# MasterXiong/Hyper-VLA

Hardware: AMD Instinct MI355X
Metric: actions_per_sec (higher is better)
Workload: dtype f16; 1 GPU; BASELINE configs[1]: hypernet weight-gen once (untimed) + full sample_actions step (u8 224x224 -> DINOv2-base E=768 in the loop -> generated vit_t 4L/64d policy -> [4,7] action chunk); 1 action = 1 sample-step; batch_per_gpu=256, global_batch=256, encoder=DINOv2-base (reference parity, E=768), parallelism=episode-dp1 (no collectives), policy_operands=split-bf16 (bf16x3), launch=eager (114 launches per step, counted by the library), streams=1, ensemble=not in the step

## Files before the change

hyper-vla_amd/csrc/api.hip:

```cpp
#include <hip/hip_runtime.h>

#include <cmath>
#include <cstdio>
#include <cstring>
#include <map>
#include <memory>
#include <mutex>
#include <string>
#include <vector>

#include "../../include/hvla.h"
#include "common.h"
#include "kernels.h"
#include "layout.h"
#include "pack.h"
#include "t5.h"
#include "train.h"

using namespace hvla;

namespace {

struct DevBuf {
  void* p = nullptr;
// ... 19 lines not shown
  DevBuf slot_count;
};

struct hvla_post {
  int B = 0, H = 0;
  DevBuf ring;
  DevBuf state;
};

struct hvla_ctx {
  hvla_config cfg{};
  Geom g{};
  int device = 0;
  std::string err;
  bool loaded = false;
  bool train_timer = false;
  PackedLayout lay;
  int Kp = 0;
  DevBuf hn_f32;
  CtxParams ctxp{};
  DevBuf wcat_hi, wcat_lo, bcat, perm;
  DevBuf enc16, encd16, encf32;
  EncWeights encw{};
  DevBuf ctx_hi, ctx_lo, ctx_f32, ws_x, ws_h, ws_qkv, ws_g, ws_corr, ws_abar, ws_lncnt, ws_lnpart, tokens, flags;
  uint32_t ln_spin = 800;
#ifdef HVLA_BENCH_HOOKS
  int enc_stop = 0;
#endif
  Profiler prof;
  float *amap_dino = nullptr, *amap_head = nullptr;
  hipStream_t side = nullptr;
  hipEvent_t ev_fork = nullptr, ev_join = nullptr;
  std::vector<hvla_weights*> arena_pool;
  std::mutex pool_mu;
  static constexpr size_t ARENA_POOL_MAX = 4;
  hipEvent_t ev_bucket[3] = {nullptr, nullptr, nullptr};
  bool bucket_recorded[3] = {false, false, false};
  ~hvla_ctx() {
    for (hvla_weights* w : arena_pool) delete w;
    for (hipEvent_t e : ev_bucket)
      if (e) (void)hipEventDestroy(e);
    if (ev_fork) (void)hipEventDestroy(ev_fork);
    if (ev_join) (void)hipEventDestroy(ev_join);
    if (side) (void)hipStreamDestroy(side);
  }
  int rs_H = 0, rs_W = 0, rs_row_span = 0, rs_col_span = 0;
  DevBuf rs_tab, rs_rows, rs_img, rs_pad;
  bool t5_loaded = false;
  T5Dims t5d{};
// ... 59 lines not shown
  ctx->Kp = 2 * ((g.patch * g.patch * 3 + 63) / 64 * 64);
  {
    std::vector<uint8_t> seen(ctx->lay.pl.G, 0);
    for (int32_t r : ctx->lay.perm)
      if (r >= 0) {
        if (r >= ctx->lay.pl.G || seen[r]) return HVLA_E_STATE;
        seen[r] = 1;
      }
    for (uint8_t s : seen)
      if (!s) return HVLA_E_STATE;
  }
  const size_t Bm = c->max_batch, S = g.S(), E = g.E, F = g.enc_mlp;
  size_t gbytes = Bm * S * F * 2;
  if (gbytes < Bm * P * ctx->Kp * 2) gbytes = Bm * P * ctx->Kp * 2;
  hipError_t e = hipSuccess;
  auto A = [&](DevBuf& b, size_t n) { if (e == hipSuccess) e = b.alloc(n); };
  A(ctx->ctx_hi, Bm * g.C * 2); A(ctx->ctx_lo, Bm * g.C * 2); A(ctx->ctx_f32, Bm * g.C * 4);
  A(ctx->ws_x, Bm * S * E * 4); A(ctx->ws_h, Bm * S * E * 2); A(ctx->ws_qkv, Bm * S * 3 * E * 2);
  A(ctx->ws_g, gbytes); A(ctx->tokens, Bm * P * E * 4); A(ctx->flags, 64 * sizeof(int));
  A(ctx->ws_corr, 2 * Bm * (F > 3 * E ? F : 3 * E) * 4);
  A(ctx->ws_abar, 2 * Bm * (F > E ? F : E) * 2);
  A(ctx->ws_lncnt, (Bm + 4) * 4 + 64);
  A(ctx->ws_lnpart, Bm * 4 * 256 * 16);
  if (e != hipSuccess) return HVLA_E_ARENA_FULL;
  if (hipMemset(ctx->ws_lncnt.p, 0, ctx->ws_lncnt.bytes) != hipSuccess) return HVLA_E_HIP;
  if (c->streams == 2) {
    if (hipStreamCreateWithFlags(&ctx->side, hipStreamNonBlocking) != hipSuccess ||
        hipEventCreateWithFlags(&ctx->ev_fork, hipEventDisableTiming) != hipSuccess ||
        hipEventCreateWithFlags(&ctx->ev_join, hipEventDisableTiming) != hipSuccess)
      return HVLA_E_HIP;
  } else if (c->streams != 0 && c->streams != 1) {
    return HVLA_E_SHAPE;
  }
  *out = ctx.release();
  return HVLA_OK;
}

void hvla_destroy(hvla_ctx* ctx) {
  if (!ctx) return;
  (void)hipSetDevice(ctx->device);
  if (ctx->train_timer) train_gemm_timer_release();
  delete ctx;
}

int64_t hvla_num_generated(const hvla_ctx* ctx) { return ctx ? ctx->lay.pl.G : 0; }

// ... 300 lines not shown
  if (context)
    HIPCHK(ctx, hipMemcpyAsync(context, w->ctx.p, (size_t)w->B * ctx->g.C * 4, hipMemcpyDeviceToDevice, st));
  return HVLA_OK;
}

static int check_step(hvla_ctx* ctx, int32_t B) {
  if (!ctx->loaded) FAIL(ctx, HVLA_E_STATE, "called before hvla_load_weights");
  if (B < 1 || B > ctx->cfg.max_batch) FAIL(ctx, HVLA_E_SHAPE, "batch %d outside [1, %d]", B, ctx->cfg.max_batch);
  return HVLA_OK;
}

static int encode_range(hvla_ctx* ctx, const uint8_t* images, float* out, int b0, int nb, bool keep_cls, hipStream_t st) {
  const Geom& g = ctx->g;
  const size_t S = g.S(), E = g.E, F = g.enc_mlp, rows = (size_t)b0 * S;
  const size_t gper = S * F > (size_t)g.P() * ctx->Kp ? S * F : (size_t)g.P() * ctx->Kp;
  EncWorkspace ws{ctx->ws_x.as<float>() + rows * E, static_cast<char*>(ctx->ws_h.p) + rows * E * 2,
                  static_cast<char*>(ctx->ws_qkv.p) + rows * 3 * E * 2, static_cast<char*>(ctx->ws_g.p) + (size_t)b0 * gper * 2,
                  ctx->ws_corr.as<float>() + (size_t)2 * b0 * (F > 3 * E ? F : 3 * E),
                  static_cast<char*>(ctx->ws_abar.p) + (size_t)2 * b0 * (F > E ? F : E) * 2};
  if (ctx->amap_dino) ws.amap = ctx->amap_dino + (size_t)b0 * g.enc_layers * g.enc_heads * g.P();
  ws.ln_cnt = ctx->ws_lncnt.as<uint32_t>() + (size_t)((b0 + 3) / 4 * 4);
  ws.ln_part = ctx->ws_lnpart.as<float>() + (size_t)b0 * 4 * 256 * 4;
  ws.ln_spin = ctx->ln_spin;
#ifdef HVLA_BENCH_HOOKS
  ws.stop_after = ctx->enc_stop;
#endif
  const size_t img = (size_t)g.image_size * g.image_size * 3, per = (keep_cls ? S : (size_t)g.P()) * E;
  HIPCHK(ctx, launch_encoder(g, ctx->cfg.enc_dtype, ctx->encw, ws, images + (size_t)b0 * img, out + (size_t)b0 * per, nb, st,
                             &ctx->prof, keep_cls));
  return HVLA_OK;
}

int hvla_encode(hvla_ctx* ctx, const uint8_t* images, float* tokens, int32_t B, void* stream) {
  if (!ctx) return HVLA_E_STATE;
  if (int r = check_step(ctx, B)) return r;
  if (!images || !tokens) FAIL(ctx, HVLA_E_SHAPE, "null pointer");
  HIPCHK(ctx, hipSetDevice(ctx->device));
  return encode_range(ctx, images, tokens, 0, B, false, reinterpret_cast<hipStream_t>(stream));
}

int hvla_encode_hidden(hvla_ctx* ctx, const uint8_t* images, float* hidden, int32_t B, void* stream) {
  if (!ctx) return HVLA_E_STATE;
  if (int r = check_step(ctx, B)) return r;
  if (!images || !hidden) FAIL(ctx, HVLA_E_SHAPE, "null pointer");
  HIPCHK(ctx, hipSetDevice(ctx->device));
  return encode_range(ctx, images, hidden, 0, B, true, reinterpret_cast<hipStream_t>(stream));
}

int hvla_encode_audit(hvla_ctx* ctx, const uint8_t* images, int32_t B, float* maxabs, int32_t* nonfinite, void* stream) {
  if (!ctx) return HVLA_E_STATE;
  if (int r = check_step(ctx, B)) return r;
  if (!images || !maxabs || !nonfinite) FAIL(ctx, HVLA_E_SHAPE, "null pointer");
  HIPCHK(ctx, hipSetDevice(ctx->device));
  hipStream_t st = reinterpret_cast<hipStream_t>(stream);
  uint32_t* slots = reinterpret_cast<uint32_t*>(ctx->flags.p);
  HIPCHK(ctx, hipMemsetAsync(slots, 0, 8 * sizeof(uint32_t), st));
  const Geom& g = ctx->g;
  const size_t F = g.enc_mlp, E = g.E;
  EncWorkspace ws{ctx->ws_x.as<float>(), ctx->ws_h.p, ctx->ws_qkv.p, ctx->ws_g.p, ctx->ws_corr.as<float>(), ctx->ws_abar.p};
  (void)F; (void)E;
  ws.ln_cnt = ctx->ws_lncnt.as<uint32_t>(); ws.ln_part = ctx->ws_lnpart.as<float>(); ws.ln_spin = ctx->ln_spin;
  HIPCHK(ctx, launch_encoder(g, ctx->cfg.enc_dtype, ctx->encw, ws, images, ctx->tokens.as<float>(), B, st, nullptr, false, slots));
  uint32_t h[8];
  HIPCHK(ctx, hipMemcpyAsync(h, slots, sizeof h, hipMemcpyDeviceToHost, st));
  HIPCHK(ctx, hipStreamSynchronize(st));
  for (int i = 0; i < 4; ++i) {
    memcpy(&maxabs[i], &h[2 * i], 4);
    nonfinite[i] = (int32_t)h[2 * i + 1];
  }
  return HVLA_OK;
}

static int policy_range(hvla_ctx* ctx, const hvla_weights* w, const float* tokens, float* actions, float* logits, int b0,
                        int nb, hipStream_t st, const int32_t* slots = nullptr) {
  const Geom& g = ctx->g;
  const PolicyLayout& pl = ctx->lay.pl;
  const size_t wb = slots ? 0 : (size_t)b0;
  PolicyParams p{pl, w->wh.as<__bf16>() + wb * pl.Gm, w->wl.as<__bf16>() + wb * pl.Gm,
                 w->vf.as<float>() + wb * pl.Gv, tokens + (size_t)b0 * g.P() * g.E,
                 actions + (size_t)b0 * g.horizon * g.action_dim, logits ? logits + (size_t)b0 * g.horizon : nullptr,
                 nb, g.E, g.P(), g.L, g.M, g.horizon, g.action_dim, g.tanh_scale, g.max_action};
  const LangLayout& ll = ctx->lay.ll;
  const int lang_T = ll.on ? g.T : 0;
  if (ctx->amap_head) p.amap = ctx->amap_head + (size_t)b0 * g.L * g.H * (g.P() + lang_T);
// ... 541 lines not shown
  HIPCHK(ctx, hipMemset(st.p, 0, (size_t)n * 8));
  PolicyParams p{pl, w->wh.as<__bf16>(), w->wl.as<__bf16>(), w->vf.as<float>(), tokens, actions, logits,
                 B, g.E, g.P(), g.L, g.M, g.horizon, g.action_dim, g.tanh_scale, g.max_action};
  p.stamps = st.as<unsigned long long>();
  for (int i = 0; i < 3; ++i) HIPCHK(ctx, launch_policy(p, nullptr));
  HIPCHK(ctx, hipDeviceSynchronize());
  HIPCHK(ctx, hipMemcpy(out, st.p, (size_t)n * 8, hipMemcpyDeviceToHost));
  return HVLA_OK;
}

int hvla_debug_train_gemm_exact(int on) {
  set_train_gemm_exact(on != 0);
  return HVLA_OK;
}
int hvla_debug_ctx_stamps(unsigned long long* out) { return debug_ctx_stamps(out) == hipSuccess ? HVLA_OK : HVLA_E_HIP; }
int hvla_debug_workspace(hvla_ctx* ctx, int which, void** ptr, size_t* bytes) {
  if (!ctx || !ptr || !bytes) return HVLA_E_STATE;
  DevBuf* b[8] = {&ctx->ws_x, &ctx->ws_h, &ctx->ws_qkv, &ctx->ws_g, &ctx->ws_corr, &ctx->ws_abar, &ctx->ws_lncnt, &ctx->ws_lnpart};
  if (which < 0 || which > 7) return HVLA_E_SHAPE;
  *ptr = b[which]->p;
  *bytes = b[which]->bytes;
  return HVLA_OK;
}
int hvla_debug_lnx_stats(hvla_ctx* ctx, unsigned long long* out, int reset) {
  if (!ctx) return HVLA_E_STATE;
  HIPCHK(ctx, hipSetDevice(ctx->device));
  HIPCHK(ctx, debug_lnx_stats(out, reset));
  return HVLA_OK;
}
int hvla_debug_encode_stop(hvla_ctx* ctx, int32_t n) {
  if (!ctx || n < 0) return HVLA_E_STATE;
  ctx->enc_stop = n;
  return HVLA_OK;
}
int hvla_debug_lnx_spin(hvla_ctx* ctx, uint32_t ticks) {
  if (!ctx) return HVLA_E_STATE;
  ctx->ln_spin = ticks;
  return HVLA_OK;
}
#endif

int64_t hvla_launches(hvla_ctx* ctx) {
  if (!ctx) return 0;
  const int64_t n = (int64_t)ctx->prof.nlaunch;
  ctx->prof.nlaunch = 0;
  return n;
// ... 29 lines not shown
```

hyper-vla_amd/csrc/encoder.hip:

```cpp
#include <cstring>
#include <type_traits>

#include "common.h"
#include "kernels.h"
#include "plan.h"

namespace hvla {

template <typename Op>
__global__ void im2col_kernel(const uint8_t* __restrict__ img, typename Op::elem* __restrict__ out, int B,
                              int image, int patch, int grid, int Kp, float* __restrict__ x, const float* __restrict__ pos, int S, int E) {
  for (size_t i = (size_t)blockIdx.x * blockDim.x + threadIdx.x; i < (size_t)B * E; i += (size_t)gridDim.x * blockDim.x)
    x[(i / E) * S * E + (i % E)] = pos[i % E];
  const int Kp1 = Kp / 2, chunks = Kp1 / 8;
  const size_t total = (size_t)B * grid * grid * chunks;
  const int kreal = patch * patch * 3;
  for (size_t i = (size_t)blockIdx.x * blockDim.x + threadIdx.x; i < total; i += (size_t)gridDim.x * blockDim.x) {
    const int ch = (int)(i % chunks);
    const size_t m = i / chunks;
    const int px = (int)(m % grid), py = (int)((m / grid) % grid);
    const size_t b = m / ((size_t)grid * grid);
    typename Op::x8 v;
    const int rowb = 3 * patch;
    const int k0 = ch * 8;
// ... 1856 lines not shown
    }
    o[((size_t)b * S + (S - 1)) * E + head * 64 + lane] = (T)last;
    if (omean) {
      const int NH = NW / 2;
      float t0 = 0.f, t1 = last;
      if (NW == 8) {
        float c[8];
#pragma unroll
        for (int w = 0; w < 8; ++w) c[w] = csum[w * 64 + lane];
#pragma unroll
        for (int w = 0; w < 4; ++w) t0 += c[w], t1 += c[4 + w];
      } else {
        for (int w = 0; w < NH; ++w) t0 += csum[w * 64 + lane];
        for (int w = NH; w < NW; ++w) t1 += csum[w * 64 + lane];
      }
      if (NH == 0) t0 = t1;
      omean[((size_t)b * 2 + 0) * E + head * 64 + lane] = (T)(t0 / (float)(NH ? NH * 32 : S));
      omean[((size_t)b * 2 + 1) * E + head * 64 + lane] = (T)(t1 / (float)(NH ? S - NH * 32 : S));
    }
  }
  HVLA_ASTAMP();
}

template <typename T>
__global__ __launch_bounds__(256) void colmean_kernel(const T* __restrict__ a, T* __restrict__ abar, int S, int P, int K) {
  typedef T T8 __attribute__((ext_vector_type(8)));
  __shared__ float part[8][256];
  const int b = blockIdx.y, chain = threadIdx.x >> 5, l32 = threadIdx.x & 31;
  const int wm = chain >> 2, pq = chain & 3;
  const int n0 = blockIdx.x * 256 + l32 * 8;
  const int half = P / 2, nq = half / 4;
  T8 p;
#pragma unroll
  for (int i = 0; i < 8; ++i) p[i] = (T)0.f;
  if (n0 < K) {
    const T* base = a + ((size_t)b * S + 1 + wm * half) * K + n0;
    for (int q = pq; q < nq; q += 16) {
      T8 v[4][4];
#pragma unroll
      for (int u = 0; u < 4; ++u)
        if (q + 4 * u < nq) {
#pragma unroll
          for (int r = 0; r < 4; ++r) v[u][r] = *reinterpret_cast<const T8*>(base + (size_t)(4 * (q + 4 * u) + r) * K);
        }
#pragma unroll
      for (int u = 0; u < 4; ++u)
// ... 49 lines not shown

#define HVLA_LAUNCH(...) do { ++pf.nlaunch; hipLaunchKernelGGL(__VA_ARGS__); } while (0)
template <typename Op>
static hipError_t run_encoder(const Geom& g, const EncWeights& w, const EncWorkspace& ws, const uint8_t* images,
                              float* tokens, int B, hipStream_t st, Profiler* prof, bool keep_cls, uint32_t* audit) {
  Profiler none;
  Profiler& pf = prof ? *prof : none;
  using T = typename Op::elem;
  constexpr int opi = std::is_same<Op, OpBF16>::value ? 1 : 0;
  const int P = g.P(), S = g.S(), E = g.E, F = g.enc_mlp, H = g.enc_heads;
  const int Kp = 2 * ((g.patch * g.patch * 3 + 63) / 64 * 64);
  const int M = B * S;
  if ((size_t)M * (size_t)(F > 3 * E ? F : 3 * E) >= (1ull << 32)) return hipErrorInvalidValue;
  const size_t gsm = (size_t)2 * (GBM + GBN) * GLD * sizeof(T);
  int dev = 0;
  hipError_t e = hipGetDevice(&dev);
  if (e != hipSuccess) return e;
  if (dev < 0 || dev >= 64) return hipErrorInvalidDevice;
  DeviceInfo& di = g_dev[dev];
  if (!di.attr[opi]) {
#define SETA(K) \
  if ((e = hipFuncSetAttribute(reinterpret_cast<const void*>(K), hipFuncAttributeMaxDynamicSharedMemorySize, 160 * 1024)) != hipSuccess) return e;
    SETA((gemm_kernel<Op, EPI_PATCH>)) SETA((gemm_kernel<Op, EPI_QKV>)) SETA((gemm_kernel<Op, EPI_GELU>))
    SETA((gemm_kernel<Op, EPI_RES>)) SETA((attention_kernel<Op, false>)) SETA((attention_kernel<Op, true>)) SETA((attention_kernel<Op, false, 8>))
    SETA((gemm256p_kernel<Op, EPI_PATCH, false>)) SETA((gemm256p_kernel<Op, EPI_QKV, false>))
    SETA((gemm256p_kernel<Op, EPI_GELU, false>)) SETA((gemm256p_kernel<Op, EPI_RES, false>))
    SETA((gemm256p_kernel<Op, EPI_PATCH, true>)) SETA((gemm256p_kernel<Op, EPI_QKV, true>))
    SETA((gemm256p_kernel<Op, EPI_GELU, true>)) SETA((gemm256p_kernel<Op, EPI_RES, true>))
    SETA((gemm256p_kernel<Op, EPI_PATCH, false, true>)) SETA((gemm256p_kernel<Op, EPI_RES, false, true>))
    SETA((gemm256p_kernel<Op, EPI_PATCH, true, true>)) SETA((gemm256p_kernel<Op, EPI_RES, true, true>))
    SETA((gemm256p_kernel<Op, EPI_RES, false, true, true>)) SETA((gemm256p_kernel<Op, EPI_RES, true, true, true>))
    SETA((gemm64_kernel<Op, EPI_PATCH>)) SETA((gemm64_kernel<Op, EPI_QKV>)) SETA((gemm64_kernel<Op, EPI_GELU>))
    SETA((gemm64_kernel<Op, EPI_RES>)) SETA((gemm64_kernel<Op, EPI_CORR>))
    SETA((gemm64_kernel<Op, EPI_QKV, 4>)) SETA((gemm64_kernel<Op, EPI_GELU, 4>)) SETA((gemm64_kernel<Op, EPI_RES, 4>))
    SETA((gemm64c_kernel<Op, EPI_QKV>)) SETA((gemm64c_kernel<Op, EPI_GELU>)) SETA((gemm64c_kernel<Op, EPI_RES>)) SETA((gemm64c32_kernel<Op>))
    SETA((gemm64c_kernel<Op, EPI_QKV, true>)) SETA((gemm64c_kernel<Op, EPI_GELU, true>)) SETA((layernorm_group_kernel<Op>))
    SETA((gemm256p_kernel<Op, EPI_QKV, false, false, true>)) SETA((gemm256p_kernel<Op, EPI_GELU, false, false, true>))
    SETA((gemm256p_kernel<Op, EPI_QKV, true, false, true>)) SETA((gemm256p_kernel<Op, EPI_GELU, true, false, true>))
    SETA((gemm256p_kernel<Op, EPI_RES, false, false, true>)) SETA((gemm256p_kernel<Op, EPI_RES, true, false, true>))
#undef SETA
    di.attr[opi] = true;
  }
  if (!di.ncu && (hipDeviceGetAttribute(&di.ncu, hipDeviceAttributeMultiprocessorCount, dev) != hipSuccess || di.ncu <= 0)) di.ncu = 256;
  const int ncu = di.ncu;
  constexpr int G64_MAXM = 2047;
  constexpr int CAT_COMP = 8;
  const bool comp = w.layer[0].dqkv != nullptr && ws.corr && ws.abar;
// ... 125 lines not shown
    float* partial = comp && room ? reinterpret_cast<float*>(scratch) : nullptr;
    HVLA_LAUNCH((layernorm_group_kernel<Op>), dim3(LNG, B), dim3(LNW * 64), (size_t)(P / 8) * E * sizeof(float), st, ws.x,
                       reinterpret_cast<T*>(ws.h), sc, bi, partial, S, P, E);
    if (!partial) return;
    if (small_fused(Nnext, E) && gemm64c_fold_lds(E) <= 160 * 1024 && ((M + SBM - 1) / SBM) * (Nnext / SBN) <= ncu) {
      ln_partial = partial;
      return;
    }
    HVLA_LAUNCH((layernorm_mean_kernel<Op>), dim3(2 * B), dim3(256), 0, st, partial, reinterpret_cast<T*>(ws.abar), P, E);
  };
  auto colmean_of = [&](const void* act, int K) {
    if (!comp) return;
    HVLA_LAUNCH((colmean_kernel<T>), dim3((K + 255) / 256, B), dim3(256), 0, st, reinterpret_cast<const T*>(act),
                       reinterpret_cast<T*>(ws.abar), S, P, K);
  };
  auto audit_of = [&](const void* buf, size_t n, int site) {
    if (!audit) return;
    HVLA_LAUNCH((absmax_kernel<T>), dim3(1024), dim3(256), 0, st, reinterpret_cast<const T*>(buf), n / 8, audit + 2 * site);
  };
  if (can_fuse_ln && P == HBM_ && M > G64_MAXM) {
    if ((e = hipMemsetAsync(ws.ln_cnt, 0, (size_t)((B * 4 + 15) / 16 * 16), st)) != hipSuccess) return e;
    if ((e = hipMemsetAsync(ws.ln_part, 0, (size_t)B * ((E + HBN_ - 1) / HBN_) * 256 * 16, st)) != hipSuccess) return e;
    pf.nlaunch += 2;
  }
  using EQ = std::integral_constant<int, EPI_QKV>;
  using EG = std::integral_constant<int, EPI_GELU>;
  using ER = std::integral_constant<int, EPI_RES>;
  pf.begin(0, st);
  {
    const size_t total = (size_t)B * P * (Kp / 16);
    int blocks = (int)((total + 255) / 256);
    if (blocks > 8192) blocks = 8192;
    HVLA_LAUNCH(im2col_kernel<Op>, dim3(blocks), dim3(256), 0, st, images, reinterpret_cast<T*>(ws.g), B,
                       g.image_size, g.patch, g.grid(), Kp, ws.x, w.pos, S, E);
    const int Mp = B * P;
    GemmArgs a{ws.g, w.w_patch, Mp, E, Kp, w.b_patch, w.pos, ws.x, P, S, 0, 1.f / 256.f};
    const bool fits32 = (size_t)Mp * Kp < (1ull << 31);
    if (Mp % HBM_ == 0 && E % SBN == 0 && E >= HBN_ && Mp > G64_MAXM && fits32) {
      a.nbm = Mp / HBM_; a.tile_row0 = 0; a.tile_stride = HBM_;
      const int nbn = (E + HBN_ - 1) / HBN_;
      if (P == HBM_ && can_fuse_ln && g.enc_layers > 0) {
        a.hsplit = hsplit;
        lnx_args(a, w.layer[0].ln1_s, w.layer[0].ln1_b, nbn);
        if (lnx_persistent(a.nbm, nbn)) HVLA_LAUNCH((gemm256p_kernel<Op, EPI_PATCH, true, true>), dim3(ncu), dim3(512), 131072, st, a);
        else HVLA_LAUNCH((gemm256p_kernel<Op, EPI_PATCH, false, true>), dim3(a.nbm * nbn), dim3(512), 131072, st, a);
        ln_fused = true;
// ... 19 lines not shown
    const EncLayerW& L = w.layer[l];
    if (!ln_fused) {
      pf.begin(1, st);
      layernorm(L.ln1_s, L.ln1_b, 3 * E, ws.g, F);
      pf.end(1, st);
    }
    audit_of(ws.h, (size_t)M * E, 0);
    gemm(EQ{}, ws.h, L.wqkv, L.dqkv, 3 * E, E, L.bqkv, nullptr, ws.qkv, E, 2);
    audit_of(ws.qkv, (size_t)M * 3 * E, 1);
    HVLA_STOP_HERE();
    pf.begin(3, st);
    const bool att_unrolled = KT == 9;
    auto attn = [&](auto kern, size_t lds) {
      HVLA_LAUNCH(kern, dim3(B * H), dim3((KT - 1) * 64), lds, st, reinterpret_cast<const T*>(ws.qkv), reinterpret_cast<T*>(ws.h), S, E, H,
                  comp ? reinterpret_cast<T*>(ws.abar) : nullptr, ws.amap ? ws.amap + (size_t)l * H * (S - 1) : nullptr, g.enc_layers * H * (S - 1)
#ifdef HVLA_BENCH_HOOKS
                  , (unsigned long long*)nullptr, 0
#endif
                  );
    };
    if (ws.amap) {
      attn(attention_kernel<Op, true>, asm_bytes + (size_t)(KT * 32 + 32) * sizeof(float));
    } else {
      if (att_unrolled) attn(attention_kernel<Op, false, 8>, asm_bytes);
      else attn(attention_kernel<Op, false>, asm_bytes);
    }
    pf.end(3, st);
    audit_of(ws.h, (size_t)M * E, 2);
    gemm(ER{}, ws.h, L.wo, L.dwo, E, E, L.bo, L.ls1, ws.x, 0, 4, nullptr, L.ln2_s, L.ln2_b);
    if (!ln_fused) {
      pf.begin(1, st);
      layernorm(L.ln2_s, L.ln2_b, F, ws.qkv, 3 * E);
      pf.end(1, st);
    }
    HVLA_STOP_HERE();
    audit_of(ws.h, (size_t)M * E, 0);
    const bool summed = gemm(EG{}, ws.h, L.w1, L.dw1, F, E, L.b1, nullptr, ws.g, 0, 5, comp ? ws.abar : nullptr);
    audit_of(ws.g, (size_t)M * F, 3);
    if (!summed) colmean_of(ws.g, F);
    HVLA_STOP_HERE();
    if (l + 1 < g.enc_layers) gemm(ER{}, ws.g, L.w2, L.dw2, E, F, L.b2, L.ls2, ws.x, 0, 6, nullptr, w.layer[l + 1].ln1_s, w.layer[l + 1].ln1_b);
    else gemm(ER{}, ws.g, L.w2, L.dw2, E, F, L.b2, L.ls2, ws.x, 0, 6);
    HVLA_STOP_HERE();
  }
#undef HVLA_STOP_HERE
  pf.begin(1, st);
  if (keep_cls)
// ... 41 lines not shown
    else if (variant == 2) hipLaunchKernelGGL((gemm256p_kernel<Op, EPI, false>), dim3(nt), dim3(512), 131072, st, a);
    else hipLaunchKernelGGL((gemm256p_kernel<Op, EPI, true>), dim3(nt < ncu ? nt : ncu), dim3(512), 131072, st, a);
  };
  auto launch = [&]() {
    if (epi == EPI_QKV) launch_e(std::integral_constant<int, EPI_QKV>{});
    else if (epi == EPI_GELU) launch_e(std::integral_constant<int, EPI_GELU>{});
    else launch_e(std::integral_constant<int, EPI_RES>{});
  };
  hipEvent_t e0, e1;
  (void)hipEventCreate(&e0);
  (void)hipEventCreate(&e1);
  launch();
  (void)hipEventRecord(e0, st);
  for (int i = 0; i < iters; ++i) launch();
  (void)hipEventRecord(e1, st);
  (void)hipEventSynchronize(e1);
  (void)hipEventElapsedTime(ms, e0, e1);
  *ms /= iters;
  (void)hipEventDestroy(e0);
  (void)hipEventDestroy(e1);
  return hipGetLastError();
}
hipError_t debug_attention_stamps(const void* qkv, void* o, void* omean, int B, int S, int E, int H, int wg, unsigned long long* stamps,
                                  hipStream_t st) {
  using Op = OpF16;
  using T = Op::elem;
  const int KT = (S + 31) / 32;
  const size_t asm_bytes = (size_t)KT * 32 * 2 * AVLD * sizeof(T) + (size_t)KT * APS * sizeof(float) + 64 * sizeof(T) +
                           (size_t)(KT - 1) * 64 * sizeof(float);
  auto go = [&](auto kern) {
    (void)hipFuncSetAttribute(reinterpret_cast<const void*>(kern), hipFuncAttributeMaxDynamicSharedMemorySize, 160 * 1024);
    hipLaunchKernelGGL(kern, dim3(B * H), dim3((KT - 1) * 64), asm_bytes, st, reinterpret_cast<const T*>(qkv),
                       reinterpret_cast<T*>(o), S, E, H, reinterpret_cast<T*>(omean), (float*)nullptr, 0, stamps, wg);
  };
  if (KT == 9) go(attention_kernel<Op, false, 8>);
  else go(attention_kernel<Op, false>);
  return hipGetLastError();
}
#endif

hipError_t launch_encoder(const Geom& g, int dtype, const EncWeights& w, const EncWorkspace& ws,
                          const uint8_t* images, float* tokens, int B, hipStream_t st, Profiler* prof, bool keep_cls,
                          uint32_t* audit) {
  if (dtype == 1) return run_encoder<OpBF16>(g, w, ws, images, tokens, B, st, prof, keep_cls, audit);
  return run_encoder<OpF16>(g, w, ws, images, tokens, B, st, prof, keep_cls, audit);
}

}
```

hyper-vla_amd/csrc/kernels.h:

```cpp
#pragma once
#include <hip/hip_runtime.h>
#include <stdint.h>

#include <vector>

#include "../../include/hvla.h"
#include "layout.h"

namespace hvla {

struct CtxLayer {
  const float *ln0_s, *ln0_b, *wq, *bq, *wk, *bk, *wv, *bv, *wo, *bo, *ln1_s, *ln1_b, *w1, *b1, *w2, *b2;
};
constexpr int CTX_MAX_LAYERS = 8;
struct CtxParams {
  int T, C, F, heads, layers, lang_dim, E, scale_context;
  int big_elems;
  const float* tok;
  const int64_t* attn_mask;
  const float* cls;
  const float *w_tok, *b_tok, *w_img, *b_img, *pos_tok, *pos_img, *pos_layer, *norm_s, *norm_b;
  CtxLayer layer[CTX_MAX_LAYERS];
  float* ctx;
  __bf16 *ctx_hi, *ctx_lo;
// ... 19 lines not shown
  const void *wqkv, *wo, *w1, *w2;
  const void *dqkv, *dwo, *dw1, *dw2;
  const float *bqkv, *bo, *b1, *b2;
  const float *ln1_s, *ln1_b, *ln2_s, *ln2_b, *ls1, *ls2;
};
constexpr int ENC_MAX_LAYERS = 24;
struct EncWeights {
  const void* w_patch;
  const float* b_patch;
  const float* pos;
  const float *lnf_s, *lnf_b;
  EncLayerW layer[ENC_MAX_LAYERS];
};
struct EncWorkspace {
  float* x;
  void* h;
  void* qkv;
  void* g;
  float* corr;
  void* abar;
  float* amap = nullptr;
  uint32_t* ln_cnt = nullptr;
  float* ln_part = nullptr;
  uint32_t ln_spin = 800;
#ifdef HVLA_BENCH_HOOKS
  int stop_after = 0;
#endif
};
struct Profiler {
  int mode = 0;
  uint32_t select = 1u << 5;
  std::vector<hipEvent_t> start, stop;
  std::vector<int> cat;
  size_t used = 0;
  uint64_t nlaunch = 0;
  bool want(int c) const { return c >= 0 && (mode == 2 || (mode == 1 && ((select >> c) & 1u))); }
  void begin(int c, hipStream_t st) {
    if (!want(c)) return;
    if (used == start.size()) {
      hipEvent_t a, b;
      if (hipEventCreate(&a) != hipSuccess || hipEventCreate(&b) != hipSuccess) return;
      start.push_back(a), stop.push_back(b), cat.push_back(c);
    }
    cat[used] = c;
    (void)hipEventRecord(start[used], st);
  }
  void end(int c, hipStream_t st) {
    if (!want(c) || used >= start.size()) return;
    (void)hipEventRecord(stop[used], st);
    ++used;
  }
};
hipError_t launch_encoder(const Geom& g, int dtype, const EncWeights& w, const EncWorkspace& ws,
                          const uint8_t* images, float* tokens, int B, hipStream_t st, Profiler* prof,
                          bool keep_cls = false,
                          uint32_t* audit = nullptr);

#ifdef HVLA_BENCH_HOOKS
hipError_t debug_gemm(const void* A, const void* W, const float* bias, const float* aux, void* out, int M, int N,
                      int K, int epi, int variant, int iters, float* ms, hipStream_t st);
hipError_t debug_lnx_stats(unsigned long long* out, int reset);
hipError_t debug_ctx_stamps(unsigned long long* out);
hipError_t debug_attention_stamps(const void* qkv, void* o, void* omean, int B, int S, int E, int H, int wg, unsigned long long* stamps,
                                  hipStream_t st);
#endif

void build_resize_spans(int in_size, int out_size, std::vector<int>& start, std::vector<int>& count, std::vector<float>& w,
                        int& maxspan);
hipError_t launch_resize(const uint8_t* src, uint8_t* dst, float* tmp_rows, float* tmp_img, const int* row_start,
                         const int* row_count, const float* row_w, int row_span, const int* col_start, const int* col_count,
                         const float* col_w, int col_span, int B, int H, int W, int S, int crop, hipStream_t st,
                         float* padded = nullptr, int src_h = 0, int src_w = 0);

struct PolicyParams {
  PolicyLayout pl;
  const __bf16 *wh, *wl;
  const float* vf;
  const float* tokens;
  float* actions;
  float* logits;
  int B, E, P, L, M, horizon, action_dim;
  float tanh_scale, max_action;
  float* amap = nullptr;
#ifdef HVLA_BENCH_HOOKS
  unsigned long long* stamps = nullptr;
#endif
};
// ... 44 lines not shown
```

Before: 18670 actions/s.

## Add persistent work-queue attention kernel overlapping next item's K/V loads

Adds a persistent DINOv2 attention kernel that launches at most two workgroups per CU. Each workgroup pulls (batch, head) items from an atomic ticket queue and prefetches the next item's Q/K/V into LDS while it computes the current one. The kernel is used by default when S==257, there is no attention-map capture, and B*H exceeds the slot count. The goal is to remove per-workgroup launch and tail overhead and hide global load latency. In exchange it adds one memset launch per encode, hand-tuned vmcnt waits and inline asm that are fragile, and an always-present queue buffer.

```diff
diff --git a/hyper-vla_amd/csrc/api.hip b/hyper-vla_amd/csrc/api.hip
--- a/hyper-vla_amd/csrc/api.hip
+++ b/hyper-vla_amd/csrc/api.hip
@@ -65,9 +65,10 @@
   DevBuf wcat_hi, wcat_lo, bcat, perm;
   DevBuf enc16, encd16, encf32;
   EncWeights encw{};
-  DevBuf ctx_hi, ctx_lo, ctx_f32, ws_x, ws_h, ws_qkv, ws_g, ws_corr, ws_abar, ws_lncnt, ws_lnpart, tokens, flags;
+  DevBuf ctx_hi, ctx_lo, ctx_f32, ws_x, ws_h, ws_qkv, ws_g, ws_corr, ws_abar, ws_lncnt, ws_lnpart, ws_attq, tokens, flags;
   uint32_t ln_spin = 800;
 #ifdef HVLA_BENCH_HOOKS
+  int att_form = 0;
   int enc_stop = 0;
 #endif
   Profiler prof;
@@ -173,6 +174,7 @@
   A(ctx->ws_abar, 2 * Bm * (F > E ? F : E) * 2);
   A(ctx->ws_lncnt, (Bm + 4) * 4 + 64);
   A(ctx->ws_lnpart, Bm * 4 * 256 * 16);
+  A(ctx->ws_attq, 2 * ENC_MAX_LAYERS * sizeof(uint32_t));
   if (e != hipSuccess) return HVLA_E_ARENA_FULL;
   if (hipMemset(ctx->ws_lncnt.p, 0, ctx->ws_lncnt.bytes) != hipSuccess) return HVLA_E_HIP;
   if (c->streams == 2) {
@@ -519,8 +521,10 @@
   ws.ln_cnt = ctx->ws_lncnt.as<uint32_t>() + (size_t)((b0 + 3) / 4 * 4);
   ws.ln_part = ctx->ws_lnpart.as<float>() + (size_t)b0 * 4 * 256 * 4;
   ws.ln_spin = ctx->ln_spin;
+  ws.att_queue = ctx->ws_attq.as<uint32_t>() + (b0 ? ENC_MAX_LAYERS : 0);
 #ifdef HVLA_BENCH_HOOKS
   ws.stop_after = ctx->enc_stop;
+  ws.att_form = ctx->att_form;
 #endif
   const size_t img = (size_t)g.image_size * g.image_size * 3, per = (keep_cls ? S : (size_t)g.P()) * E;
   HIPCHK(ctx, launch_encoder(g, ctx->cfg.enc_dtype, ctx->encw, ws, images + (size_t)b0 * img, out + (size_t)b0 * per, nb, st,
@@ -557,6 +561,7 @@
   EncWorkspace ws{ctx->ws_x.as<float>(), ctx->ws_h.p, ctx->ws_qkv.p, ctx->ws_g.p, ctx->ws_corr.as<float>(), ctx->ws_abar.p};
   (void)F; (void)E;
   ws.ln_cnt = ctx->ws_lncnt.as<uint32_t>(); ws.ln_part = ctx->ws_lnpart.as<float>(); ws.ln_spin = ctx->ln_spin;
+  ws.att_queue = ctx->ws_attq.as<uint32_t>();
   HIPCHK(ctx, launch_encoder(g, ctx->cfg.enc_dtype, ctx->encw, ws, images, ctx->tokens.as<float>(), B, st, nullptr, false, slots));
   uint32_t h[8];
   HIPCHK(ctx, hipMemcpyAsync(h, slots, sizeof h, hipMemcpyDeviceToHost, st));
@@ -1144,6 +1149,32 @@
   *bytes = b[which]->bytes;
   return HVLA_OK;
 }
+int hvla_debug_attention_form(hvla_ctx* ctx, int32_t form) {
+  if (!ctx || form < 0 || form > 2) return HVLA_E_STATE;
+  ctx->att_form = form;
+  return HVLA_OK;
+}
+int hvla_debug_attention_persist(hvla_ctx* ctx, int32_t B, int32_t wg, unsigned long long* stamps, unsigned long long* pace, int32_t* grid) {
+  if (!ctx || !stamps || !pace || !grid) return HVLA_E_STATE;
+  HIPCHK(ctx, hipSetDevice(ctx->device));
+  const Geom& g = ctx->g;
+  int ncu = 256;
+  HIPCHK(ctx, hipDeviceGetAttribute(&ncu, hipDeviceAttributeMultiprocessorCount, ctx->device));
+  const int n = B * g.enc_heads < 2 * ncu ? B * g.enc_heads : 2 * ncu;
+  DevBuf st, pc;
+  HIPCHK(ctx, st.alloc((size_t)16 * 8 * 8));
+  HIPCHK(ctx, pc.alloc((size_t)n * 2 * 8));
+  for (int rep = 0; rep < 2; ++rep) {
+    HIPCHK(ctx, hipMemset(st.p, 0, st.bytes));
+    HIPCHK(ctx, debug_attention_stamps(ctx->ws_qkv.p, ctx->ws_h.p, ctx->ws_abar.p, B, g.S(), g.E, g.enc_heads, wg, st.as<unsigned long long>(), nullptr, 1,
+                                       ctx->ws_attq.as<uint32_t>(), pc.as<unsigned long long>()));
+    HIPCHK(ctx, hipDeviceSynchronize());
+  }
+  HIPCHK(ctx, hipMemcpy(stamps, st.p, st.bytes, hipMemcpyDeviceToHost));
+  HIPCHK(ctx, hipMemcpy(pace, pc.p, pc.bytes, hipMemcpyDeviceToHost));
+  *grid = n;
+  return HVLA_OK;
+}
 int hvla_debug_lnx_stats(hvla_ctx* ctx, unsigned long long* out, int reset) {
   if (!ctx) return HVLA_E_STATE;
   HIPCHK(ctx, hipSetDevice(ctx->device));
diff --git a/hyper-vla_amd/csrc/encoder.hip b/hyper-vla_amd/csrc/encoder.hip
--- a/hyper-vla_amd/csrc/encoder.hip
+++ b/hyper-vla_amd/csrc/encoder.hip
@@ -1902,6 +1902,383 @@
   HVLA_ASTAMP();
 }
 
+template <typename Op>
+__global__ void attention_persist_kernel(const typename Op::elem* __restrict__ qkv, typename Op::elem* __restrict__ o,
+                                         int E, int H, int nitems, typename Op::elem* __restrict__ omean,
+                                         uint32_t* __restrict__ queue
+#ifdef HVLA_BENCH_HOOKS
+                                         , unsigned long long* stamps = nullptr
+                                         , int stamp_wg = 0
+                                         , unsigned long long* pace = nullptr
+#endif
+                                         ) {
+  using T = typename Op::elem;
+  using X8 = typename Op::x8;
+  constexpr int S = 257, NW = 8, KT = 9, SP = KT * 32;
+  extern __shared__ __attribute__((aligned(16))) char smem[];
+  T* Ks = reinterpret_cast<T*>(smem);
+  T* Vs = Ks + SP * AVLD;
+  T* qxs = Vs + SP * AVLD;
+  float* part = reinterpret_cast<float*>(qxs + 128);
+  float* csum = part + KT * APS;
+  const int tid = threadIdx.x, wave = tid >> 6, lane = tid & 63;
+  const size_t rowstride = (size_t)3 * E;
+  const int col = lane & 31, half = lane >> 5;
+  const int q = wave * 32 + col;
+#ifdef HVLA_BENCH_HOOKS
+  int nstamp = 0, kitem = 0;
+  unsigned long long t_first = 0;
+#define HVLA_PSTAMP() do { if (stamps && (int)blockIdx.x == stamp_wg && tid == 0 && kitem < 16) stamps[kitem * 8 + nstamp] = __builtin_readcyclecounter(); ++nstamp; } while (0)
+  if (pace && tid == 0) t_first = __builtin_readcyclecounter();
+#else
+#define HVLA_PSTAMP() do { } while (0)
+#endif
+  auto base_of = [&](int it) { return qkv + (size_t)(it / H) * S * rowstride + (it % H) * 64; };
+  X8 qf[4];
+  auto opaque = [](int v) { asm volatile("" : "+v"(v)); return v; };
+  auto load_q = [&](const T* bs) {
+    const int le = opaque(lane);
+    const uint32_t qo = (uint32_t)(((size_t)(wave * 32 + (le & 31)) * rowstride + (le >> 5) * 8) * sizeof(T));
+    asm volatile("global_load_dwordx4 %0, %4, %5\n\tglobal_load_dwordx4 %1, %4, %5 offset:32\n\t"
+                 "global_load_dwordx4 %2, %4, %5 offset:64\n\tglobal_load_dwordx4 %3, %4, %5 offset:96"
+                 : "=&v"(qf[0]), "=&v"(qf[1]), "=&v"(qf[2]), "=&v"(qf[3]) : "v"(qo), "s"(bs) : "memory");
+  };
+  const int rho = tid >> 3, slot = tid & 7;
+  const int ksrc = kperm(rho);
+  const uint32_t ko = (uint32_t)(((size_t)ksrc * rowstride + E + ((slot ^ (ksrc & 7)) * 8)) * sizeof(T));
+  const uint32_t vo = (uint32_t)(((size_t)rho * rowstride + 2 * E + ((slot ^ (((rho >> 1) & 1) << 2)) * 8)) * sizeof(T));
+  const uint32_t lds0 = (uint32_t)(uintptr_t)(__attribute__((address_space(3))) char*)smem;
+  const uint32_t kl = __builtin_amdgcn_readfirstlane(lds0 + wave * 1024), vl = kl + (uint32_t)(SP * AVLD * sizeof(T));
+  const uint32_t qxl = lds0 + (uint32_t)(2 * SP * AVLD * sizeof(T));
+  auto dma = [&](const T* bs, uint32_t off, uint32_t dst) {
+    uint32_t keep;
+    asm volatile("s_mov_b32 %0, m0\n\ts_mov_b32 m0, %3\n\ts_nop 0\n\tglobal_load_lds_dwordx4 %1, %2 nt\n\ts_mov_b32 m0, %0"
+                 : "=&s"(keep) : "v"(off), "s"(bs), "s"(dst) : "memory");
+  };
+  auto chunk = [&](const T* bs, int c) {
+    dma(bs + (size_t)c * 64 * rowstride, ko, kl + c * 8192);
+    dma(bs + (size_t)c * 64 * rowstride, vo, vl + c * 8192);
+  };
+  auto park = [&](const T* bs, int buf) {
+    if (lane < 8) dma(bs + (size_t)(S - 1) * rowstride - E, ko, qxl + buf * 128);
+  };
+  uint32_t tk;
+  auto ticket = [&] {
+    const uint32_t zero = 0, one = 1;
+    uint64_t keep;
+    asm volatile("s_mov_b64 %1, exec\n\ts_mov_b64 exec, 1\n\tglobal_atomic_add %0, %2, %3, %4 sc0\n\ts_mov_b64 exec, %1"
+                 : "=&v"(tk), "=&s"(keep) : "v"(zero), "v"(one), "s"(queue) : "memory");
+  };
+  auto hand_over = [&] {
+    __builtin_amdgcn_sched_barrier(0);
+    __builtin_amdgcn_s_barrier();
+    asm volatile("" ::: "memory");
+    __builtin_amdgcn_sched_barrier(0);
+  };
+#define HVLA_VMWAIT(N) asm volatile("s_waitcnt vmcnt(%0)" :: "n"(N) : "memory")
+  int item = blockIdx.x;
+  const T* base = base_of(item);
+  int par = 0;
+  bool first = true;
+  if (wave == 0) ticket();
+  load_q(base);
+  if (wave == 0) park(base, 0);
+#pragma unroll
+  for (int c = 0; c < 4; ++c) chunk(base, c);
+  if (tid >= 8 && tid < 256) {
+    X8 z;
+#pragma unroll
+    for (int j = 0; j < 8; ++j) z[j] = (T)0.f;
+    *reinterpret_cast<X8*>(Ks + (256 + rho) * AVLD + slot * 8) = z;
+    *reinterpret_cast<X8*>(Vs + (256 + rho) * AVLD + slot * 8) = z;
+  }
+  HVLA_VMWAIT(6);
+  asm volatile("" : "+v"(qf[0]), "+v"(qf[1]), "+v"(qf[2]), "+v"(qf[3]));
+  if (wave == 0) {
+    asm volatile("" : "+v"(tk));
+    const int second = (int)(gridDim.x + __builtin_amdgcn_readfirstlane(tk));
+    if (lane == 0) reinterpret_cast<int*>(part)[APS + 2] = second;
+  }
+  asm volatile("s_waitcnt lgkmcnt(0)" ::: "memory");
+
+  const int g16 = lane >> 4, i16 = lane & 15;
+  const int vsw = ((i16 >> 3) & 1) << 5;
+  const T* vtr = Vs + ((g16 >> 1) * 4 + (i16 >> 2)) * AVLD + (g16 & 1) * 16 + (i16 & 3) * 4;
+  const int kswz = col & 7;
+  const int colp = kperm(col);
+  auto kfrag = [&](int kt, int ks) {
+    return *reinterpret_cast<const X8*>(Ks + (kt * 32 + colp) * AVLD + (((2 * ks + half) ^ kswz) * 8));
+  };
+  auto zero16 = [] {
+    f32x16 z;
+#pragma unroll
+    for (int r = 0; r < 16; ++r) z[r] = 0.f;
+    return z;
+  };
+  auto mask16 = [&] {
+    f32x16 z;
+#pragma unroll
+    for (int r = 0; r < 16; ++r) z[r] = ((KT - 1) * 32 + crow(r, half) < S) ? 0.f : -1e30f;
+    return z;
+  };
+  auto qk = [&](int kt, f32x16 c) {
+#pragma unroll
+    for (int ks = 0; ks < 4; ++ks) c = Op::mma32(kfrag(kt, ks), qf[ks], c);
+    return c;
+  };
+  typedef float f32x2v __attribute__((ext_vector_type(2)));
+  auto half_exchange_max = [](float t) {
+    float u = t;
+    asm("s_nop 1\n\tv_permlane32_swap_b32 %0, %1" : "+v"(t), "+v"(u));
+    return fmaxf(t, u);
+  };
+  auto half_exchange_sum = [](float t) {
+    float u = t;
+    asm("s_nop 1\n\tv_permlane32_swap_b32 %0, %1" : "+v"(t), "+v"(u));
+    return t + u;
+  };
+  auto tile_max = [&](const f32x16& sc) {
+    float t = sc[0];
+#pragma unroll
+    for (int r = 1; r < 16; ++r) t = fmaxf(t, sc[r]);
+    float u = t;
+    asm("s_nop 1\n\tv_permlane32_swap_b32 %0, %1" : "+v"(t), "+v"(u));
+    return __builtin_ceilf(fmaxf(t, u));
+  };
+
+  for (;;) {
+    hand_over();
+    HVLA_PSTAMP();
+    float mx = -1e30f;
+    f32x2v lsum2 = {0.f, 0.f};
+    f32x16 O[2];
+#pragma unroll
+    for (int r = 0; r < 16; ++r) O[0][r] = 0.f, O[1][r] = 0.f;
+    auto pv = [&](int kt, const f32x16& sc) {
+      X8 pf[2];
+      {
+        const float tm = tile_max(sc);
+        if (kt == 0) {
+          mx = tm;
+        } else if (__builtin_amdgcn_ballot_w64(tm > mx + 8.f) != 0) {
+          const float mn = fmaxf(mx, tm);
+          const float al = __builtin_amdgcn_exp2f(mx - mn);
+#pragma unroll
+          for (int r = 0; r < 16; ++r) O[0][r] *= al, O[1][r] *= al;
+          lsum2[0] *= al, lsum2[1] *= al;
+          mx = mn;
+        }
+      }
+#pragma unroll
+      for (int r = 0; r < 16; r += 2) {
+        const f32x2v p2 = {__builtin_amdgcn_exp2f(sc[r] - mx), __builtin_amdgcn_exp2f(sc[r + 1] - mx)};
+        { float la = lsum2[0], lb = lsum2[1];
+          la += p2[0]; asm volatile("" : "+v"(la));
+          lb += p2[1]; asm volatile("" : "+v"(lb));
+          lsum2[0] = la, lsum2[1] = lb; }
+        pf[r >> 3][r & 7] = (T)p2[0];
+        pf[r >> 3][(r & 7) + 1] = (T)p2[1];
+      }
+#pragma unroll
+      for (int mt = 0; mt < 2; ++mt) {
+#pragma unroll
+        for (int sstep = 0; sstep < 2; ++sstep) {
+          const T* v0 = vtr + ((kt * 32 + sstep * 16) * AVLD) + ((mt * 32) ^ vsw);
+          O[mt] = Op::mma32(tr_read2<X8>(v0, v0 + 8 * AVLD), pf[sstep], O[mt]);
+        }
+      }
+    };
+    const T* qx = qxs + par * 64;
+    auto lastq = [&](int tile) {
+      f32x16 c = zero16();
+#pragma unroll
+      for (int ks = 0; ks < 4; ++ks) c = Op::mma32(kfrag(tile, ks), *reinterpret_cast<const X8*>(qx + ks * 16 + half * 8), c);
+      float m = c[0];
+#pragma unroll
+      for (int r = 1; r < 16; ++r) m = fmaxf(m, c[r]);
+      m = half_exchange_max(m);
+      X8 pf[2];
+      float la = 0.f, lb = 0.f;
+#pragma unroll
+      for (int r = 0; r < 16; r += 2) {
+        const float p0 = __builtin_amdgcn_exp2f(c[r] - m), p1 = __builtin_amdgcn_exp2f(c[r + 1] - m);
+        la += p0; asm volatile("" : "+v"(la));
+        lb += p1; asm volatile("" : "+v"(lb));
+        pf[r >> 3][r & 7] = (T)p0;
+        pf[r >> 3][(r & 7) + 1] = (T)p1;
+      }
+      float l = la + lb;
+      l = half_exchange_sum(l);
+      float* pp = part + tile * APS;
+      if (col == 0 && half == 0) pp[0] = m, pp[1] = l;
+#pragma unroll
+      for (int mt = 0; mt < 2; ++mt) {
+        f32x16 ol = zero16();
+#pragma unroll
+        for (int sstep = 0; sstep < 2; ++sstep) {
+          const T* v0 = vtr + ((tile * 32 + sstep * 16) * AVLD) + ((mt * 32) ^ vsw);
+          ol = Op::mma32(tr_read2<X8>(v0, v0 + 8 * AVLD), pf[sstep], ol);
+        }
+        if (col == 0) {
+#pragma unroll
+          for (int g4 = 0; g4 < 4; ++g4)
+            *reinterpret_cast<f32x4*>(pp + 4 + 32 * mt + 8 * g4 + 4 * half) = f32x4{ol[4 * g4], ol[4 * g4 + 1], ol[4 * g4 + 2], ol[4 * g4 + 3]};
+        }
+        __builtin_amdgcn_sched_barrier(0);
+      }
+    };
+    pv(0, qk(0, zero16()));
+    pv(1, qk(1, zero16()));
+    if ((wave >> 1) == 0) lastq(wave);
+    if (first) HVLA_VMWAIT(4); else HVLA_VMWAIT(16);
+    hand_over();
+    const int nxt = __builtin_amdgcn_readfirstlane(reinterpret_cast<const int*>(part)[(par ^ 1) * APS + 2]);
+    const bool hn = nxt < nitems;
+    const T* nbase = base_of(hn ? nxt : item);
+    if (wave == 0) {
+      if (lane < 8) dma(base + (size_t)256 * rowstride, ko, kl + 4 * 8192);
+      if (hn) ticket();
+    } else if (wave == 4) {
+      if (lane < 8) dma(base + (size_t)224 * rowstride, vo, vl - 4 * 1024 + 4 * 8192);
+    }
+    if (hn) {
+      chunk(nbase, 0);
+      if (wave == 0) park(nbase, par ^ 1);
+    }
+    pv(2, qk(2, zero16()));
+    pv(3, qk(3, zero16()));
+    if ((wave >> 1) == 1) lastq(wave);
+    if (first) { if (hn) HVLA_VMWAIT(4); else HVLA_VMWAIT(2); }
+    else { if (hn) HVLA_VMWAIT(16); else HVLA_VMWAIT(14); }
+    hand_over();
+    if (hn) chunk(nbase, 1);
+    pv(4, qk(4, zero16()));
+    pv(5, qk(5, zero16()));
+    if ((wave >> 1) == 2) lastq(wave);
+    if (first) { if (hn) HVLA_VMWAIT(4); else HVLA_VMWAIT(0); }
+    else { if (hn) HVLA_VMWAIT(16); else HVLA_VMWAIT(12); }
+    hand_over();
+    if (hn) chunk(nbase, 2);
+    pv(6, qk(6, zero16()));
+    pv(7, qk(7, zero16()));
+    if ((wave >> 1) == 3) lastq(wave);
+    if (!hn) HVLA_VMWAIT(0);
+    else if (wave == 0) HVLA_VMWAIT(7);
+    else HVLA_VMWAIT(6);
+    if (wave == 0 && hn) {
+      asm volatile("" : "+v"(tk));
+      const int third = (int)(gridDim.x + __builtin_amdgcn_readfirstlane(tk));
+      if (lane == 0) reinterpret_cast<int*>(part)[par * APS + 2] = third;
+    }
+    hand_over();
+    HVLA_PSTAMP();
+    if (hn) chunk(nbase, 3);
+    {
+      const f32x16 sc8 = qk(KT - 1, mask16());
+      __builtin_amdgcn_sched_barrier(0);
+      load_q(nbase);
+      __builtin_amdgcn_sched_barrier(0);
+      pv(KT - 1, sc8);
+    }
+    if (wave == 0) {
+      const int key = S - 1, le = opaque(lane);
+      const float sc = wave64_sum((float)qx[le] * (float)Ks[kperm(key) * AVLD + (((le >> 3) ^ (key & 7)) * 8) + (le & 7)]);
+      float* pp = part + (KT - 1) * APS;
+      if (le == 0) pp[0] = sc, pp[1] = 1.f;
+      pp[4 + le] = (float)Vs[key * AVLD + (le ^ (((key >> 1) & 1) << 5))];
+    }
+    const float inv = 1.f / half_exchange_sum(lsum2[0] + lsum2[1]);
+    HVLA_PSTAMP();
+    const int b = item / H, head = item % H;
+    {
+      const int le = opaque(lane), half = le >> 5;
+      T* op = o + ((size_t)b * S * E + head * 64) + (uint32_t)((wave * 32 + (le & 31)) * E + half * 4);
+      float w16[16];
+#pragma unroll
+      for (int j = 0; j < 16; ++j) O[0][j] *= inv, O[1][j] *= inv;
+#pragma unroll
+      for (int mt = 0; mt < 2; ++mt)
+#pragma unroll
+        for (int g4 = 0; g4 < 4; ++g4) {
+          typename Op::x4 v4;
+#pragma unroll
+          for (int r = 0; r < 4; ++r) v4[r] = (T)O[mt][g4 * 4 + r];
+          *reinterpret_cast<typename Op::x4*>(op + mt * 32 + g4 * 8) = v4;
+        }
+      if (omean) {
+#pragma unroll
+        for (int j = 0; j < 16; j += 4) {
+          float a0 = O[0][j], a1 = O[0][j + 1], a2 = O[0][j + 2], a3 = O[0][j + 3];
+          float b0 = O[1][j], b1 = O[1][j + 1], b2 = O[1][j + 2], b3 = O[1][j + 3];
+          asm("s_nop 1\n\tv_permlane16_swap_b32 %0, %4\n\tv_permlane16_swap_b32 %1, %5\n\tv_permlane16_swap_b32 %2, %6\n\tv_permlane16_swap_b32 %3, %7"
+              : "+v"(a0), "+v"(a1), "+v"(a2), "+v"(a3), "+v"(b0), "+v"(b1), "+v"(b2), "+v"(b3));
+          w16[j] = a0 + b0, w16[j + 1] = a1 + b1, w16[j + 2] = a2 + b2, w16[j + 3] = a3 + b3;
+        }
+        const bool b3 = le & 8, b2 = le & 4, b1 = le & 2, b0 = le & 1;
+        float w8[8], w4[4], w2[2];
+#pragma unroll
+        for (int j = 0; j < 8; ++j) w8[j] = (b3 ? w16[j + 8] : w16[j]) + dpp_mov<0x140>(b3 ? w16[j] : w16[j + 8]);
+#pragma unroll
+        for (int j = 0; j < 4; ++j) w4[j] = (b2 ? w8[j + 4] : w8[j]) + dpp_mov<0x141>(b2 ? w8[j] : w8[j + 4]);
+#pragma unroll
+        for (int j = 0; j < 2; ++j) w2[j] = (b1 ? w4[j + 2] : w4[j]) + dpp_mov<0x4E>(b1 ? w4[j] : w4[j + 2]);
+        const float w1 = (b0 ? w2[1] : w2[0]) + dpp_mov<0xB1>(b0 ? w2[0] : w2[1]);
+        const int j = le & 31;
+        csum[wave * 64 + (j >> 4) * 32 + ((j >> 2) & 3) * 8 + half * 4 + (j & 3)] = w1;
+      }
+    }
+    HVLA_PSTAMP();
+    asm volatile("s_waitcnt lgkmcnt(0)" ::: "memory");
+    hand_over();
+    HVLA_PSTAMP();
+    if (wave == 0) {
+      const int le = opaque(lane);
+      float pm[KT], pl[KT], po[KT];
+#pragma unroll
+      for (int t = 0; t < KT; ++t) {
+        pm[t] = part[t * APS];
+        pl[t] = part[t * APS + 1];
+        po[t] = part[t * APS + 4 + le];
+      }
+      float M = -1e30f;
+#pragma unroll
+      for (int t = 0; t < KT; ++t) M = fmaxf(M, pm[t]);
+      float L = 0.f, od = 0.f;
+#pragma unroll
+      for (int t = 0; t < KT; ++t) {
+        const float f = __builtin_amdgcn_exp2f(pm[t] - M);
+        L = fmaf(pl[t], f, L);
+        od = fmaf(po[t], f, od);
+      }
+      const float last = od / L;
+      o[((size_t)b * S + (S - 1)) * E + head * 64 + le] = (T)last;
+      if (omean) {
+        float t0 = 0.f, t1 = last;
+        float c[8];
+#pragma unroll
+        for (int w = 0; w < 8; ++w) c[w] = csum[w * 64 + le];
+#pragma unroll
+        for (int w = 0; w < 4; ++w) t0 += c[w], t1 += c[4 + w];
+        omean[((size_t)b * 2 + 0) * E + head * 64 + le] = (T)(t0 / (float)(4 * 32));
+        omean[((size_t)b * 2 + 1) * E + head * 64 + le] = (T)(t1 / (float)(S - 4 * 32));
+      }
+    }
+    HVLA_PSTAMP();
+#ifdef HVLA_BENCH_HOOKS
+    ++kitem, nstamp = 0;
+#endif
+    if (!hn) break;
+    item = nxt, base = nbase, par ^= 1, first = false;
+    HVLA_VMWAIT(8);
+    asm volatile("" : "+v"(qf[0]), "+v"(qf[1]), "+v"(qf[2]), "+v"(qf[3]));
+  }
+#ifdef HVLA_BENCH_HOOKS
+  if (pace && tid == 0) pace[blockIdx.x * 2] = (unsigned long long)kitem, pace[blockIdx.x * 2 + 1] = __builtin_readcyclecounter() - t_first;
+#endif
+#undef HVLA_VMWAIT
+#undef HVLA_PSTAMP
+}
+
 template <typename T>
 __global__ __launch_bounds__(256) void colmean_kernel(const T* __restrict__ a, T* __restrict__ abar, int S, int P, int K) {
   typedef T T8 __attribute__((ext_vector_type(8)));
@@ -1997,7 +2374,7 @@
 #define SETA(K) \
   if ((e = hipFuncSetAttribute(reinterpret_cast<const void*>(K), hipFuncAttributeMaxDynamicSharedMemorySize, 160 * 1024)) != hipSuccess) return e;
     SETA((gemm_kernel<Op, EPI_PATCH>)) SETA((gemm_kernel<Op, EPI_QKV>)) SETA((gemm_kernel<Op, EPI_GELU>))
-    SETA((gemm_kernel<Op, EPI_RES>)) SETA((attention_kernel<Op, false>)) SETA((attention_kernel<Op, true>)) SETA((attention_kernel<Op, false, 8>))
+    SETA((gemm_kernel<Op, EPI_RES>)) SETA((attention_kernel<Op, false>)) SETA((attention_kernel<Op, true>)) SETA((attention_kernel<Op, false, 8>)) SETA((attention_persist_kernel<Op>))
     SETA((gemm256p_kernel<Op, EPI_PATCH, false>)) SETA((gemm256p_kernel<Op, EPI_QKV, false>))
     SETA((gemm256p_kernel<Op, EPI_GELU, false>)) SETA((gemm256p_kernel<Op, EPI_RES, false>))
     SETA((gemm256p_kernel<Op, EPI_PATCH, true>)) SETA((gemm256p_kernel<Op, EPI_QKV, true>))
@@ -2169,6 +2546,16 @@
     if ((e = hipMemsetAsync(ws.ln_cnt, 0, (size_t)((B * 4 + 15) / 16 * 16), st)) != hipSuccess) return e;
     if ((e = hipMemsetAsync(ws.ln_part, 0, (size_t)B * ((E + HBN_ - 1) / HBN_) * 256 * 16, st)) != hipSuccess) return e;
     pf.nlaunch += 2;
+  }
+  const int att_slots = 2 * ncu;
+  bool att_persist = ws.att_queue != nullptr && S == 257 && !ws.amap && B * H > att_slots && g.enc_layers > 0;
+#ifdef HVLA_BENCH_HOOKS
+  if (ws.att_form == 1) att_persist = false;
+  else if (ws.att_form == 2) att_persist = ws.att_queue != nullptr && S == 257 && !ws.amap && g.enc_layers > 0;
+#endif
+  if (att_persist) {
+    if ((e = hipMemsetAsync(ws.att_queue, 0, (size_t)g.enc_layers * sizeof(uint32_t), st)) != hipSuccess) return e;
+    pf.nlaunch += 1;
   }
   using EQ = std::integral_constant<int, EPI_QKV>;
   using EG = std::integral_constant<int, EPI_GELU>;
@@ -2234,7 +2621,15 @@
     if (ws.amap) {
       attn(attention_kernel<Op, true>, asm_bytes + (size_t)(KT * 32 + 32) * sizeof(float));
     } else {
-      if (att_unrolled) attn(attention_kernel<Op, false, 8>, asm_bytes);
+      if (att_persist)
+        HVLA_LAUNCH((attention_persist_kernel<Op>), dim3(B * H < att_slots ? B * H : att_slots), dim3(512), asm_bytes + 64 * sizeof(T), st,
+                    reinterpret_cast<const T*>(ws.qkv), reinterpret_cast<T*>(ws.h), E, H, B * H, comp ? reinterpret_cast<T*>(ws.abar) : nullptr,
+                    ws.att_queue + l
+#ifdef HVLA_BENCH_HOOKS
+                    , (unsigned long long*)nullptr, 0, (unsigned long long*)nullptr
+#endif
+                    );
+      else if (att_unrolled) attn(attention_kernel<Op, false, 8>, asm_bytes);
       else attn(attention_kernel<Op, false>, asm_bytes);
     }
     pf.end(3, st);
@@ -2322,12 +2717,24 @@
   return hipGetLastError();
 }
 hipError_t debug_attention_stamps(const void* qkv, void* o, void* omean, int B, int S, int E, int H, int wg, unsigned long long* stamps,
-                                  hipStream_t st) {
+                                  hipStream_t st, int form, uint32_t* queue, unsigned long long* pace) {
   using Op = OpF16;
   using T = Op::elem;
   const int KT = (S + 31) / 32;
   const size_t asm_bytes = (size_t)KT * 32 * 2 * AVLD * sizeof(T) + (size_t)KT * APS * sizeof(float) + 64 * sizeof(T) +
                            (size_t)(KT - 1) * 64 * sizeof(float);
+  if (form == 1) {
+    if (S != 257 || !queue) return hipErrorInvalidValue;
+    int dev = 0, ncu = 256;
+    (void)hipGetDevice(&dev);
+    (void)hipDeviceGetAttribute(&ncu, hipDeviceAttributeMultiprocessorCount, dev);
+    hipError_t e = hipFuncSetAttribute(reinterpret_cast<const void*>(attention_persist_kernel<Op>), hipFuncAttributeMaxDynamicSharedMemorySize, 160 * 1024);
+    if (e != hipSuccess) return e;
+    if ((e = hipMemsetAsync(queue, 0, sizeof(uint32_t), st)) != hipSuccess) return e;
+    hipLaunchKernelGGL((attention_persist_kernel<Op>), dim3(B * H < 2 * ncu ? B * H : 2 * ncu), dim3(512), asm_bytes + 64 * sizeof(T), st,
+                       reinterpret_cast<const T*>(qkv), reinterpret_cast<T*>(o), E, H, B * H, reinterpret_cast<T*>(omean), queue, stamps, wg, pace);
+    return hipGetLastError();
+  }
   auto go = [&](auto kern) {
     (void)hipFuncSetAttribute(reinterpret_cast<const void*>(kern), hipFuncAttributeMaxDynamicSharedMemorySize, 160 * 1024);
     hipLaunchKernelGGL(kern, dim3(B * H), dim3((KT - 1) * 64), asm_bytes, st, reinterpret_cast<const T*>(qkv),
diff --git a/hyper-vla_amd/csrc/kernels.h b/hyper-vla_amd/csrc/kernels.h
--- a/hyper-vla_amd/csrc/kernels.h
+++ b/hyper-vla_amd/csrc/kernels.h
@@ -65,9 +65,11 @@
   float* amap = nullptr;
   uint32_t* ln_cnt = nullptr;
   float* ln_part = nullptr;
+  uint32_t* att_queue = nullptr;
   uint32_t ln_spin = 800;
 #ifdef HVLA_BENCH_HOOKS
   int stop_after = 0;
+  int att_form = 0;
 #endif
 };
 struct Profiler {
@@ -105,7 +107,7 @@
 hipError_t debug_lnx_stats(unsigned long long* out, int reset);
 hipError_t debug_ctx_stamps(unsigned long long* out);
 hipError_t debug_attention_stamps(const void* qkv, void* o, void* omean, int B, int S, int E, int H, int wg, unsigned long long* stamps,
-                                  hipStream_t st);
+                                  hipStream_t st, int form = 0, uint32_t* queue = nullptr, unsigned long long* pace = nullptr);
 #endif
 
 void build_resize_spans(int in_size, int out_size, std::vector<int>& start, std::vector<int>& count, std::vector<float>& w,
```

New measurement: 18320 actions/s. 1.9% lower.
